# hamzalsheikh/multi-cluster-simulator

Measured on AMD Instinct MI355X. Metric: job placements/sec (whole node) at 4096 clusters x 256 nodes, higher is better.
Workload: dtype u32; 1 GPU; C4: 4096 clusters total x 256 nodes, split 4096 per GPU over 1 GPU(s) (strong sharding, clusters keyed by global index), FIFO, no trading, 16384 jobs/cluster, scaled per-second Poisson arrivals at 90% memory load (lambda=1.5386/s); clusters_total=4096, clusters_per_gpu=4096, nodes=256, jobs_per_cluster=16384, gen=stream, max_dur=600, parallelism=dp1: one system's clusters split over the GPUs, no collective on the data path

## Files before the change

### multi-cluster-simulator_amd/csrc/mcs_fa_macros.h

```cpp
#pragma once


#define MCS_FA_PRIO(P)                                                                            \
    "s_sub_u32 s76, s42, s57\n\t"                                                                 \
    "s_cselect_b32 s76, 0, s76\n\t"                                                               \
    "s_lshl_b32 s76, s76, 1\n\t"                                                                  \
    "s_cmp_gt_u32 s76, s42\n\t"                                                                   \
    "s_cbranch_scc0 " P "p2_%=\n\t"                                                              \
    "s_setprio 3\n\t"                                                                            \
    "s_branch " P "pe_%=\n"                                                                       \
    P "p2_%=:\n\t"                                                                               \
    "s_lshl_b32 s76, s76, 1\n\t"                                                                  \
    "s_cmp_gt_u32 s76, s42\n\t"                                                                   \
    "s_cbranch_scc0 " P "p1_%=\n\t"                                                              \
    "s_setprio 2\n\t"                                                                            \
    "s_branch " P "pe_%=\n"                                                                       \
    P "p1_%=:\n\t"                                                                               \
    "s_lshl_b32 s76, s76, 1\n\t"                                                                  \
    "s_cmp_gt_u32 s76, s42\n\t"                                                                   \
    "s_cbranch_scc0 " P "p0_%=\n\t"                                                              \
    "s_setprio 1\n\t"                                                                            \
    "s_branch " P "pe_%=\n"                                                                       \
    P "p0_%=:\n\t"                                                                               \
    "s_setprio 0\n"                                                                               \
// ... 297 lines not shown
#define MCS_FA_ANYFIT "v_cmp_ne_u32_e32 vcc, 0, v86\n\t"
#define MCS_FA_ANYFIT32 MCS_FA_ANYFIT
#define MCS_FA_ANYFIT16 MCS_FA_ANYFIT
#define MCS_FA_ANYFIT16R MCS_FA_ANYFIT
#define MCS_FA_PICK1 "v_readlane_b32 s51, v86, s50\n\t"
#define MCS_FA_PICK2 "s_ff1_i32_b32 s52, s51\n\t"
#define MCS_FA_PICK132 MCS_FA_PICK1
#define MCS_FA_PICK116 MCS_FA_PICK1
#define MCS_FA_PICK116R MCS_FA_PICK1
#define MCS_FA_PICK232 MCS_FA_PICK2
#define MCS_FA_PICK216 MCS_FA_PICK2
#define MCS_FA_PICK216R MCS_FA_PICK2
#define MCS_FA_ZEROKX                                                                             \
    "v_readlane_b32 s51, v86, s50\n\t"                                                           \
    "s_mov_b32 m0, s47\n\t"                                                                      \
    "s_ff1_i32_b32 s52, s51\n\t"                                                                 \
    "s_lshl3_add_u32 s54, s52, s50\n\t"
#define MCS_FA_ZEROKX32 MCS_FA_ZEROKX
#define MCS_FA_ZEROKX16 MCS_FA_ZEROKX
#define MCS_FA_ZEROKX16R MCS_FA_ZEROKX
#define MCS_FA_GUARD0_                                                                            \
    "s_mov_b32 s78, 0\n\t"                                                                        \
    "s_lshl2_add_u32 s79, s42, 0x100\n\t"
#define MCS_FA_GUARD032 MCS_FA_GUARD0_
#define MCS_FA_GUARD016 MCS_FA_GUARD0_
#define MCS_FA_GUARD016S MCS_FA_GUARD0_
#define MCS_FA_HEAD32 ""
#define MCS_FA_HEAD16 ""
#define MCS_FA_HEAD16S ""
#define MCS_FA_XWAITED_ "s_mov_b32 %[waited], s82\n\t"
#define MCS_FA_XWAITED32 MCS_FA_XWAITED_
#define MCS_FA_XWAITED16 MCS_FA_XWAITED_
#define MCS_FA_XWAITED16S MCS_FA_XWAITED_
#define MCS_FA_POOLMAX32 "64*8"
#define MCS_FA_POOLMAX16 "64*8"
#define MCS_FA_POOLMAX16R "64*8"
#define MCS_FA_NODEIDX                                                                            \
    "v_and_b32 v126, 63, v91\n\t"                                                                \
    "v_lshrrev_b32 v127, 6, v91\n\t"                                                             \
    "v_lshl_add_u32 v126, v126, 2, v127\n\t"
#define MCS_FA_NODEIDX32 MCS_FA_NODEIDX
#define MCS_FA_NODEIDX16 MCS_FA_NODEIDX
#define MCS_FA_NODEIDX16R MCS_FA_NODEIDX

#define MCS_FA_FIT16C                                                                             \
    "v_pk_sub_u16 v72, v64, s48\n\t"                                                              \
    "v_pk_sub_u16 v73, v65, s48\n\t"                                                              \
    "v_pk_sub_u16 v74, v66, s48\n\t"                                                              \
    "v_pk_sub_u16 v75, v67, s48\n\t"                                                              \
    "v_and_b32_sdwa v80, v72, v72 dst_sel:WORD_0 dst_unused:UNUSED_PAD src0_sel:WORD_1 src1_sel:WORD_0\n\t" \
    "v_and_b32_sdwa v81, v74, v74 dst_sel:WORD_0 dst_unused:UNUSED_PAD src0_sel:WORD_1 src1_sel:WORD_0\n\t" \
    "v_and_b32_sdwa v80, v73, v73 dst_sel:WORD_1 dst_unused:UNUSED_PRESERVE src0_sel:WORD_1 src1_sel:WORD_0\n\t" \
    "v_and_b32_sdwa v81, v75, v75 dst_sel:WORD_1 dst_unused:UNUSED_PRESERVE src0_sel:WORD_1 src1_sel:WORD_0\n\t" \
    "s_add_u32 s55, s40, s46\n\t"     \
    "v_perm_b32 v86, v81, v80, s72\n\t"
#define MCS_FA_REC16C MCS_FA_REC16
#define MCS_FA_ZMASK16C(SRC)                                                                      \
    "v_mov_b32 v87, " SRC "\n\t"                                                                  \
    "v_cmp_eq_u32_e32 vcc, 0, v95\n\t"                                                            \
    "v_cndmask_b32_e32 v94, " SRC ", v111, vcc\n\t"
#define MCS_FA_TAKE16C                                                                            \
    "v_mov_b32 v95, v99\n\t"                                                                      \
    "v_min_u32 v96, 0x7fff, v100\n\t"                                                             \
    "v_min_u32 v97, 0x7fff, v101\n\t"                                                             \
    "v_lshl_or_b32 v96, v97, 16, v96\n\t" MCS_FA_ZMASK16C("v98")
#define MCS_FC_SHIFT                                                                              \
    "v_cmp_le_u32_e32 vcc, s41, v110\n\t"                                                         \
    "v_cndmask_b32_e32 v94, v94, v111, vcc\n\t"                                  \
    "v_mov_b32 v89, -1\n\t"                                                                       \
    "v_mov_b32 v90, 0\n\t"                                                                        \
    "v_mov_b32 v107, 0\n\t"                                                                       \
    "s_nop 1\n\t"                                                                                 \
    "v_mov_b32_dpp v89, v94 wave_shl:1 row_mask:0xf bank_mask:0xf\n\t"                            \
    "v_mov_b32_dpp v90, v95 wave_shl:1 row_mask:0xf bank_mask:0xf\n\t"                            \
    "v_mov_b32_dpp v107, v96 wave_shl:1 row_mask:0xf bank_mask:0xf\n\t"
#define MCS_FC_RECNEXT                                                                            \
    "v_readlane_b32 s45, v89, m0\n\t"                                                             \
    "v_readlane_b32 s46, v90, m0\n\t"                                                             \
    "v_readlane_b32 s48, v107, m0\n\t"
#define MCS_FA_RELOAD16C "ds_read_b128 v[64:67], v108\n\t"
#define MCS_FA_ZEROKX16C                                                                          \
    "v_readlane_b32 s51, v86, s50\n\t"                                                           \
    "s_mov_b32 m0, s47\n\t"                                                                      \
    "s_ff1_i32_b32 s52, s51\n\t"                                                                 \
    "s_lshr_b32 s53, s52, 3\n\t"                                                                 \
    "s_lshl2_add_u32 s54, s50, s53\n\t"
#define MCS_FA_POOLMAX16C "64*8"
#define MCS_FA_NODEIDX16C "v_mov_b32 v126, v91\n\t"
#define MCS_FA_XWAITED16C                                                                         \
    "s_cmp_lg_u32 s43, 0\n\t"                                                                     \
    "s_addc_u32 %[waited], s82, 0\n\t"
#define MCS_FA_GUARD016C "s_lshl2_add_u32 s78, s42, 0x100\n\t"
#define MCS_FA_HEAD16C ""
#define MCS_FA_INIT16C MCS_FA_ZMASK16C("v94")                                      \
    "s_min_u32 s41, s42, 64\n\t" MCS_FC_SHIFT                                                     \
    "s_mov_b64 s[86:87], -1\n\t"                                                                 \
    "s_mov_b64 s[88:89], -1\n\t"                                                                 \
    "s_mov_b64 s[90:91], -1\n\t"                                                                 \
    "s_mov_b64 s[92:93], -1\n\t"                                                                 \
    "s_mov_b64 s[94:95], -1\n\t"                                                                 \
    "s_mov_b64 s[96:97], -1\n\t"                                                                 \
    "s_mov_b64 s[98:99], -1\n\t"                                                                 \
    "s_mov_b64 s[100:101], -1\n\t"                                                               \
    "s_getpc_b64 s[58:59]\n"                                                                      \
    "mcsfa_pc_%=:\n\t"                                                                            \
    "s_add_u32 s74, s58, mcsfa_tbl_%=-mcsfa_pc_%=\n\t"                                           \
    "s_addc_u32 s59, s59, 0\n\t"                                                                      \
    "v_mov_b32 v32, -1\n\t"                                                                      \
    "v_mov_b32 v33, -1\n\t"                                                                      \
    "v_mov_b32 v34, -1\n\t"                                                                      \
    "v_mov_b32 v35, -1\n\t"                                                                      \
    "v_mov_b32 v36, -1\n\t"                                                                      \
    "v_mov_b32 v37, -1\n\t"                                                                      \
    "v_mov_b32 v38, -1\n\t"                                                                      \
    "v_mov_b32 v39, -1\n\t"                                                                      \
    "v_mov_b32 v106, -1\n\t"
#define MCS_FA_DECIDE16C                                                                          \
    "v_readlane_b32 s51, v86, s50\n\t"                                                            \
    "s_lshl_b64 exec, 1, s50\n\t"                                                                 \
    "s_ff1_i32_b32 s52, s51\n\t"                                                                  \
    "s_lshr_b32 s53, s52, 3\n\t"                                                                  \
    "s_lshl2_add_u32 s54, s50, s53\n\t"              \
    "s_set_gpr_idx_on s53, gpr_idx(SRC0,DST)\n\t"                                                 \
    "v_mov_b32 v64, v72\n\t"                                 \
    "s_set_gpr_idx_off\n\t"
#define MCS_FC_BREL(P, k, F, PAY, A, FREE, TAIL)                                                  \
    "mcsfa_" P #k "_%=:\n\t"                                                                      \
    "ds_write_b128 v108, v[64:67]\n\t"                                                           \
    "s_mov_b64 exec, vcc\n\t"                                                                     \
    "s_bcnt1_i32_b64 s76, vcc\n\t"                                                               \
    "v_lshl_add_u32 v121, v91, 2, v109\n\t"                                                      \
    "ds_add_u32 v121, v96\n\t"                                                                    \
    "v_mov_b32 v106, -1\n\t"                                                                      \
    "s_mov_b64 exec, -1\n\t"                                                                      \
    "v_cmp_ge_u32_e32 vcc, s40, " F "\n\t"                                                       \
    "s_cbranch_vccz mcsfa_" TAIL #k "_%=\n\t"                                                     \
    "s_mov_b64 exec, vcc\n\t"                                                                     \
    "s_bcnt1_i32_b64 s49, vcc\n\t"                                                               \
    "ds_add_u32 " A ", " PAY "\n\t"                                                             \
    "v_mov_b32 " F ", -1\n\t"                                                                    \
    "s_or_b64 " FREE ", " FREE ", vcc\n\t"                                                       \
    "s_add_u32 s76, s76, s49\n\t"                                                                 \
    "s_branch mcsfa_" TAIL #k "_%=\n"
#define MCS_FC_BMA(r, OP, ON, FREE)                                                               \
    "v_cmp_eq_u32_e64 s[60:61], " #r ", v122\n\t"                                                 \
    "s_bcnt1_i32_b64 s76, s[60:61]\n\t"                                                           \
    "v_mbcnt_lo_u32_b32 v120, s60, v121\n\t"                                                      \
    "s_bcnt1_i32_b64 s75, " FREE "\n\t"                                                           \
    "v_mbcnt_hi_u32_b32 v120, s61, v120\n\t"                                                      \
    "s_add_u32 " ON ", " OP ", s76\n\t"                                                           \
    "v_cndmask_b32_e64 v123, v123, v120, s[60:61]\n\t"                                            \
    "s_cmp_gt_u32 s76, s75\n\t"                                                                   \
    "s_cbranch_scc1 mcsfa_bmo" #r "_%=\n"                                                         \
    "mcsfa_bmr" #r "_%=:\n\t"                                                                     \
    "v_mov_b32 v121, " ON "\n\t"
#define MCS_FC_BMO(r, OP)                                                                         \
    "mcsfa_bmo" #r "_%=:\n\t"                                                                     \
    "s_add_u32 s75, s75, " OP "\n\t"                                                              \
    "v_cmp_le_u32_e32 vcc, s75, v120\n\t"                                                         \
    "s_and_b64 vcc, vcc, s[60:61]\n\t"                                                            \
    "s_or_b64 s[46:47], s[46:47], vcc\n\t"                                                        \
    "s_branch mcsfa_bmr" #r "_%=\n"
#define MCS_FC_BMB(OP, ON, FREELO, FREEHI, FREE, Q)                                               \
    "v_mov_b32 v121, " OP "\n\t"                                                                  \
    "v_mbcnt_lo_u32_b32 v120, " FREELO ", v121\n\t"                                               \
    "v_mbcnt_hi_u32_b32 v120, " FREEHI ", v120\n\t"                                               \
    "v_cmp_gt_u32_e64 s[60:61], " ON ", v120\n\t"                                                 \
    "v_lshl_add_u32 v120, v120, 4, v109\n\t"                                                      \
    "s_and_b64 exec, s[60:61], " FREE "\n\t"                                                      \
    "ds_read_b128 " Q ", v120 offset:1024\n\t"                                                    \
    "s_andn2_b64 " FREE ", " FREE ", exec\n\t"                                                    \
    "s_mov_b64 exec, -1\n\t"
#define MCS_FC_BMC(Q0, Q1, Q2, F, P, A)                                                           \
    "v_cmp_ne_u32_e32 vcc, -1, " Q0 "\n\t"                                                        \
    "v_cndmask_b32_e32 " F ", " F ", " Q0 ", vcc\n\t"                                             \
    "v_cndmask_b32_e32 " P ", " P ", " Q1 ", vcc\n\t"                                             \
    "v_cndmask_b32_e32 " A ", " A ", " Q2 ", vcc\n\t"
#define MCS_FC_BMOVE                                                                              \
    "v_cmp_ne_u32_e32 vcc, -1, v106\n\t"                                                          \
    "s_cbranch_vccz mcsfa_bmx_%=\n\t"                                                             \
    "v_and_b32 v122, 7, v106\n\t"                                                                 \
    "s_mov_b64 s[48:49], vcc\n\t"                                            \
    "v_cndmask_b32_e32 v122, 8, v122, vcc\n\t"                      \
    "s_mov_b64 s[46:47], 0\n\t"                                                                   \
    "v_mov_b32 v112, v106\n\t"                                                                    \
    "v_mov_b32 v113, v96\n\t"                                                                     \
    "v_lshl_add_u32 v114, v91, 2, v109\n\t"                                                       \
    "v_mov_b32 v121, 0\n\t"                                                                       \
    MCS_FC_BMA(0, "0", "s50", "s[86:87]") MCS_FC_BMA(1, "s50", "s51", "s[88:89]")                 \
    MCS_FC_BMA(2, "s51", "s52", "s[90:91]") MCS_FC_BMA(3, "s52", "s53", "s[92:93]")               \
    MCS_FC_BMA(4, "s53", "s54", "s[94:95]") MCS_FC_BMA(5, "s54", "s55", "s[96:97]")               \
    MCS_FC_BMA(6, "s55", "s62", "s[98:99]") MCS_FC_BMA(7, "s62", "s63", "s[100:101]")             \
    "s_mov_b64 exec, s[48:49]\n\t"                                                                \
    "v_lshl_add_u32 v123, v123, 4, v109\n\t"                                                      \
    "ds_write_b128 v123, v[112:115] offset:1024\n\t"                                              \
    "s_mov_b64 exec, -1\n\t"                                                                      \
    "v_mov_b32 v56, -1\n\t"                                                                       \
    "v_mov_b32 v60, -1\n\t"                                                                       \
    "v_mov_b32 v68, -1\n\t"                                                                       \
    "v_mov_b32 v72, -1\n\t"                                                                       \
    "v_mov_b32 v76, -1\n\t"                                                                       \
    "v_mov_b32 v82, -1\n\t"                                                                       \
    "v_mov_b32 v102, -1\n\t"                                                                      \
    "v_mov_b32 v124, -1\n\t"                                                                      \
    MCS_FC_BMB("0", "s50", "s86", "s87", "s[86:87]", "v[56:59]")                                  \
    MCS_FC_BMB("s50", "s51", "s88", "s89", "s[88:89]", "v[60:63]")                                \
    MCS_FC_BMB("s51", "s52", "s90", "s91", "s[90:91]", "v[68:71]")                                \
    MCS_FC_BMB("s52", "s53", "s92", "s93", "s[92:93]", "v[72:75]")                                \
    MCS_FC_BMB("s53", "s54", "s94", "s95", "s[94:95]", "v[76:79]")                                \
    MCS_FC_BMB("s54", "s55", "s96", "s97", "s[96:97]", "v[82:85]")                                \
    MCS_FC_BMB("s55", "s62", "s98", "s99", "s[98:99]", "v[102:105]")                              \
    MCS_FC_BMB("s62", "s63", "s100", "s101", "s[100:101]", "v[124:127]")                          \
    "s_waitcnt lgkmcnt(0)\n\t"                                                                    \
    MCS_FC_BMC("v56", "v57", "v58", "v32", "v40", "v48")                                          \
    MCS_FC_BMC("v60", "v61", "v62", "v33", "v41", "v49")                                          \
    MCS_FC_BMC("v68", "v69", "v70", "v34", "v42", "v50")                                          \
    MCS_FC_BMC("v72", "v73", "v74", "v35", "v43", "v51")                                          \
    MCS_FC_BMC("v76", "v77", "v78", "v36", "v44", "v52")                                          \
    MCS_FC_BMC("v82", "v83", "v84", "v37", "v45", "v53")                                          \
    MCS_FC_BMC("v102", "v103", "v104", "v38", "v46", "v54")                                       \
    MCS_FC_BMC("v124", "v125", "v126", "v39", "v47", "v55")                                       \
    "s_cmp_lg_u64 s[46:47], 0\n\t"                                                                \
    "s_cbranch_scc1 mcsfa_bml_%=\n"                                                               \
    "mcsfa_bmd_%=:\n\t"                                                                           \
    "v_mov_b32 v106, -1\n"                                                                        \
    "mcsfa_bmx_%=:\n\t"
#define MCS_FC_BMOVE_OOL                                                                          \
    MCS_FC_BMO(0, "0") MCS_FC_BMO(1, "s50") MCS_FC_BMO(2, "s51") MCS_FC_BMO(3, "s52")             \
    MCS_FC_BMO(4, "s53") MCS_FC_BMO(5, "s54") MCS_FC_BMO(6, "s55") MCS_FC_BMO(7, "s62")           \
    "mcsfa_bml_%=:\n\t"                                                                           \
    "s_ff1_i32_b64 s52, s[46:47]\n\t"                                                             \
    "s_lshl_b64 s[60:61], 1, s52\n\t"                                                             \
    "v_readlane_b32 s55, v106, s52\n\t"                                              \
    "v_readlane_b32 s48, v96, s52\n\t"                                              \
    "v_readlane_b32 s54, v91, s52\n\t"                                                 \
    "s_andn2_b64 s[46:47], s[46:47], s[60:61]\n\t"                                                \
    "s_and_b32 s76, s55, 7\n\t"                                                                   \
    "s_mov_b32 s49, s76\n"                                                                        \
    "mcsfa_bms_%=:\n\t"                                                                           \
    "s_add_u32 s49, s49, 1\n\t"                                                                   \
    "s_and_b32 s49, s49, 7\n\t"                                                                   \
    "s_cmp_eq_u32 s49, s76\n\t"                                                                   \
    "s_cbranch_scc1 mcsfa_poolovf_%=\n\t"                                                         \
    "s_lshl_b32 m0, s49, 1\n\t"                                                                   \
    "s_nop 0\n\t"                                                                                 \
    "s_movrels_b64 s[60:61], s[86:87]\n\t"                                                        \
    "s_cmp_lg_u64 s[60:61], 0\n\t"                                                                \
    "s_cbranch_scc0 mcsfa_bms_%=\n\t"                                                             \
    "s_ff1_i32_b64 s85, s[60:61]\n\t"                                                             \
    "s_lshl_b64 s[62:63], 1, s85\n\t"                                                             \
    "s_andn2_b64 s[50:51], s[60:61], s[62:63]\n\t"                                                \
    "s_movreld_b64 s[86:87], s[50:51]\n\t"                                                        \
    "s_min_u32 s77, s77, s55\n\t"                                                                 \
    "s_lshl2_add_u32 s79, s54, s73\n\t"                                                           \
    "s_mov_b64 exec, s[62:63]\n\t"                                                                \
    "s_set_gpr_idx_on s49, gpr_idx(DST)\n\t"                                                      \
    "v_mov_b32 v32, s55\n\t"                                                                      \
    "v_mov_b32 v40, s48\n\t"                                                                      \
    "v_mov_b32 v48, s79\n\t"                                                                      \
    "s_set_gpr_idx_off\n\t"                                                                       \
    "s_mov_b64 exec, -1\n\t"                                                                      \
    "s_cmp_lg_u64 s[46:47], 0\n\t"                                                                \
    "s_cbranch_scc1 mcsfa_bml_%=\n\t"                                                             \
    "s_branch mcsfa_bmd_%=\n"
#define MCS_FC_WMIN(DST)                                                                          \
    "s_nop 1\n\t"                                                                                 \
    "v_min_u32_dpp v120, v120, v120 row_shr:1 row_mask:0xf bank_mask:0xf\n\t"                     \
    "s_nop 1\n\t"                                                                                 \
    "v_min_u32_dpp v120, v120, v120 row_shr:2 row_mask:0xf bank_mask:0xf\n\t"                     \
    "s_nop 1\n\t"                                                                                 \
    "v_min_u32_dpp v120, v120, v120 row_shr:4 row_mask:0xf bank_mask:0xf\n\t"                     \
    "s_nop 1\n\t"                                                                                 \
    "v_min_u32_dpp v120, v120, v120 row_shr:8 row_mask:0xf bank_mask:0xf\n\t"                     \
    "s_nop 1\n\t"                                                                                 \
    "v_min_u32_dpp v120, v120, v120 row_bcast:15 row_mask:0xa bank_mask:0xf\n\t"                  \
    "s_nop 1\n\t"                                                                                 \
    "v_min_u32_dpp v120, v120, v120 row_bcast:31 row_mask:0xc bank_mask:0xf\n\t"                  \
    "s_nop 1\n\t"                                                                                 \
    "v_readlane_b32 " DST ", v120, 63\n\t"
#define MCS_FC_FROW(p, F, P, A, FREE)                                                             \
    "v_cmp_ge_u32_e32 vcc, s40, " F "\n\t"                           \
    "s_cbranch_vccz mcsfa_fr" #p "_%=\n\t"                                                       \
    "s_mov_b64 exec, vcc\n\t"                                                                     \
    "s_bcnt1_i32_b64 s76, vcc\n\t"                                                               \
    "ds_add_u32 " A ", " P "\n\t"                                                               \
    "v_mov_b32 " F ", -1\n\t"                                                                    \
    "s_add_u32 s49, s49, s76\n\t"                                                                \
    "s_or_b64 " FREE ", " FREE ", vcc\n\t"                                                       \
    "s_mov_b64 exec, -1\n"                                                    \
    "mcsfa_fr" #p "_%=:\n\t"
#define MCS_FC_XROW(p, F)                                                                         \
    "v_and_b32 v121, 7, " F "\n\t"                                                               \
    "v_cmp_ne_u32_e32 vcc, " #p ", v121\n\t"                                                     \
    "v_cndmask_b32_e32 v121, v111, " F ", vcc\n\t"                                               \
    "v_min_u32 v120, v120, v121\n\t"
#define MCS_FC_FULL                                                                               \
    "mcsfa_full_%=:\n\t"                                                                          \
    "ds_write_b128 v108, v[64:67]\n\t"                                                           \
    "s_mov_b32 s49, 0\n\t"                                                                        \
    MCS_FC_FROW(0, "v32", "v40", "v48", "s[86:87]") MCS_FC_FROW(1, "v33", "v41", "v49", "s[88:89]") \
    MCS_FC_FROW(2, "v34", "v42", "v50", "s[90:91]") MCS_FC_FROW(3, "v35", "v43", "v51", "s[92:93]") \
    MCS_FC_FROW(4, "v36", "v44", "v52", "s[94:95]") MCS_FC_FROW(5, "v37", "v45", "v53", "s[96:97]") \
    MCS_FC_FROW(6, "v38", "v46", "v54", "s[98:99]") MCS_FC_FROW(7, "v39", "v47", "v55", "s[100:101]") \
      \
    "v_cmp_ge_u32_e32 vcc, s40, v106\n\t"                                                        \
    "s_cbranch_vccz mcsfa_fr8_%=\n\t"                                                            \
    "s_mov_b64 exec, vcc\n\t"                                                                    \
    "s_bcnt1_i32_b64 s76, vcc\n\t"                                                              \
    "v_lshl_add_u32 v121, v91, 2, v109\n\t"                                                     \
    "ds_add_u32 v121, v96\n\t"                                                                   \
    "v_mov_b32 v106, -1\n\t"                                                                     \
    "s_add_u32 s49, s49, s76\n\t"                                                                \
    "s_mov_b64 exec, -1\n"                                                                       \
    "mcsfa_fr8_%=:\n\t"                                                                          \
    "s_cmp_lt_u32 s40, s77\n\t"                     \
    "s_cbranch_scc1 mcsfa_fx_%=\n\t"                                                              \
    "v_mov_b32 v120, -1\n\t"                                                                      \
    MCS_FC_XROW(0, "v32") MCS_FC_XROW(1, "v33") MCS_FC_XROW(2, "v34") MCS_FC_XROW(3, "v35")      \
    MCS_FC_XROW(4, "v36") MCS_FC_XROW(5, "v37") MCS_FC_XROW(6, "v38") MCS_FC_XROW(7, "v39")      \
    MCS_FC_WMIN("s77") "\n"                                                                      \
    "mcsfa_fx_%=:\n\t"                                                                            \
    "s_mov_b32 s76, s49\n\t"                                                                      \
    "s_cmp_eq_u32 s49, 0\n\t"                                                                     \
    "s_cbranch_scc1 mcsfa_norel_%=\n\t"                                                           \
    "s_branch mcsfa_reltail_%=\n"
#define MCS_FC_EXACTMIN                                                                           \
    "v_min3_u32 v121, v32, v33, v34\n\t"                                                         \
    "v_min3_u32 v121, v121, v35, v36\n\t"                                                        \
    "v_min3_u32 v121, v121, v37, v38\n\t"                                                        \
    "v_min3_u32 v120, v121, v39, v106\n\t" MCS_FC_WMIN("s76")
#define MCS_FC_ZROUTE(D)                                                                          \
    "mcsfa_zarr_%=:\n\t"                                                                          \
    "s_cmp_eq_u32 s47, 64\n\t"   \
    "s_cbranch_scc1 mcsfa_bend_%=\n\t"                                                            \
    "s_add_u32 s76, s57, s47\n\t"                                                                 \
    "s_cmp_ge_u32 s76, s42\n\t"                                                                   \
    "s_cbranch_scc1 mcsfa_bend_%=\n\t"                                                            \
    "v_readlane_b32 s76, v87, s47\n\t"                                     \
    "s_cmp_lg_u32 s46, 0\n\t"                                                                     \
    "s_cselect_b32 s76, s45, s76\n\t"              \
    "s_cmp_gt_u32 s76, s40\n\t"                                                                   \
    "s_cbranch_scc0 mcsfa_zfit_%=\n\t"                                                            \
    "s_sub_u32 s49, s76, s40\n\t"                                                                 \
    "s_mov_b32 s40, s76\n\t"                                       \
    MCS_FA_CNTS_##D                                                                               \
    "s_cmp_lg_u32 s49, 1\n\t"                                                                     \
    "s_cbranch_scc1 mcsfa_full_%=\n\t"                                                            \
    "s_branch mcsfa_adv1_%=\n"                                                                    \
    "mcsfa_zfit_%=:\n\t" MCS_FA_FIT16C MCS_FA_ANYFIT                                             \
    "s_cbranch_vccz mcsfa_znofit_%=\n\t"                                                          \
    "s_ff1_i32_b64 s50, vcc\n\t"                                                                  \
    "s_branch mcsfa_zero_%=\n"                                                                    \
    "mcsfa_znofit_%=:\n\t"                                                                        \
    "s_mov_b32 s43, 2\n\t"                                                                        \
    MCS_FA_CNTS_##D                                                                               \
    "s_sub_u32 s78, s78, 1\n\t"                                           \
    "s_cbranch_scc1 mcsfa_poolovf_%=\n\t"                                                         \
    "s_cmp_eq_u32 s80, 0\n\t"                                               \
    "s_cbranch_scc1 mcsfa_deadlock_%=\n\t" MCS_FC_EXACTMIN                                        \
    "s_cmp_eq_u32 s76, -1\n\t"             \
    "s_cbranch_scc1 mcsfa_poolovf_%=\n\t"                                                         \
    "s_max_u32 s40, s40, s76\n\t"                                                                 \
    "s_branch mcsfa_full_%=\n"                                                                    \
// ... 67 lines not shown
    "s_mov_b64 exec, -1\n\t"                                                                      \
    "s_sub_u32 s80, s80, s76\n\t" MCS_FA_RELOAD16C                                               \
    "s_add_u32 s55, s40, s46\n\t"                                                    \
    "s_waitcnt lgkmcnt(0)\n\t"                                                                    \
    "v_pk_sub_u16 v72, v64, s48\n\t"                                                              \
    "v_pk_sub_u16 v73, v65, s48\n\t"                                                              \
    "v_pk_sub_u16 v74, v66, s48\n\t"                                                              \
    "v_pk_sub_u16 v75, v67, s48\n\t"                                                              \
    "v_and_b32_sdwa v80, v72, v72 dst_sel:WORD_0 dst_unused:UNUSED_PAD src0_sel:WORD_1 src1_sel:WORD_0\n\t" \
    "v_and_b32_sdwa v81, v74, v74 dst_sel:WORD_0 dst_unused:UNUSED_PAD src0_sel:WORD_1 src1_sel:WORD_0\n\t" \
    "v_and_b32_sdwa v80, v73, v73 dst_sel:WORD_1 dst_unused:UNUSED_PRESERVE src0_sel:WORD_1 src1_sel:WORD_0\n\t" \
    "v_and_b32_sdwa v81, v75, v75 dst_sel:WORD_1 dst_unused:UNUSED_PRESERVE src0_sel:WORD_1 src1_sel:WORD_0\n\t" \
    "s_cmp_le_u32 s45, s40\n\t"             \
    "v_perm_b32 v86, v81, v80, s72\n\t" MCS_FA_ANYFIT                                            \
    "s_cbranch_scc1 mcsfa_fitted" #k "_%=\n\t"                                                    \
    "s_branch mcsfa_arrive" #k "_%=\n"                                                            \
    ".p2align 6\n\t"                                                                              \
    "s_nop 0\n\t"                             \
    "s_nop 0\n"                                                                                   \
                      \
    "mcsfa_norel" #k "_%=:\n"                                                                     \
    "mcsfa_inner" #k "_%=:\n\t"                                                                   \
    "s_cmp_gt_u32 s45, s40\n\t"                          \
    "s_cbranch_scc1 mcsfa_arrive" #k "_%=\n"                                                      \
    "mcsfa_fit" #k "_%=:\n\t" MCS_FA_FIT16C MCS_FA_ANYFIT "\n"                                   \
    "mcsfa_fitted" #k "_%=:\n\t"     \
    "s_cbranch_vccz mcsfa_nofit" #k "_%=\n\t"                                                     \
    "s_ff1_i32_b64 s50, vcc\n\t"                                      \
    MCS_FA_DECIDE16C                                                                              \
    "s_mov_b64 exec, -1\n\t"                                                                      \
    "s_mov_b32 m0, s47\n\t"                                                                       \
    "s_add_u32 s80, s80, 1\n\t"                                                                   \
    "v_writelane_b32 v91, s54, m0\n\t"                                                            \
    "v_writelane_b32 v92, s40, m0\n\t"                                                            \
    "v_writelane_b32 v106, s55, m0\n"                                                               \
                                                                              \
     \
                                       \
    "mcsfa_placed" #k "_%=:\n\t" MCS_FC_RECNEXT                                                  \
    "s_add_u32 s47, s47, 1\n\t"                                                                   \
    "s_cmp_le_u32 s45, s40\n\t"                                                                   \
    "s_cbranch_scc1 mcsfa_fit" #k "_%=\n\t"                                                       \
    "s_cmp_eq_u32 s45, -1\n\t"                                                                    \
    "s_cbranch_scc1 mcsfa_zarr_%=\n"                                                              \
                  \
    "mcsfa_arr2" #k "_%=:\n\t"                                                                    \
    "s_sub_u32 s76, s45, s40\n\t"                                                                 \
    "s_mov_b32 s40, s45\n\t"                                                          \
    MCS_FA_CNTS_##D                                                                               \
    "s_cmp_lg_u32 s76, 1\n\t"                                                                     \
    "s_cbranch_scc1 mcsfa_full_%=\n\t" MCS_FC_ADV(n)                                              \
                                                \
    "mcsfa_arrive" #k "_%=:\n\t"                                                                  \
    "s_cmp_eq_u32 s45, -1\n\t"       \
    "s_cbranch_scc1 mcsfa_zarr_%=\n\t"                                                            \
    "s_branch mcsfa_arr2" #k "_%=\n"                                                              \
     \
    MCS_FC_BREL("brel", k, F, P, A, FREE, "reltail") MCS_FC_BREL("wbrel", k, F, P, A, FREE, "wreltail") \
     \
     \
       \
    "mcsfa_nofit" #k "_%=:\n\t"                                                                   \
    "s_mov_b32 s43, 1\n\t"                                                                        \
    MCS_FA_CNTS_##D                                                                               \
    "s_sub_u32 s78, s78, 1\n\t"           \
    "s_cbranch_scc1 mcsfa_poolovf_%=\n\t"                                                         \
    "s_add_u32 s79, s40, 9\n\t"                                                                   \
    "s_min_u32 s79, s79, s77\n\t"                                                                 \
    "s_cmp_eq_u32 s80, 0\n\t"                                               \
    "s_cbranch_scc0 mcsfa_wsl" #n "_%=\n\t"                                                       \
    "s_branch mcsfa_deadlock_%=\n"                                                                \
          \
    "mcsfa_wnorel" #k "_%=:\n\t"                                                                  \
    "s_add_u32 s79, s40, 9\n\t"                                                                   \
    "s_min_u32 s79, s79, s77\n\t"                                                                 \
    "s_branch mcsfa_wsl" #n "_%=\n"                                                               \
      \
      \
    "mcsfa_wrel" #k "_%=:\n\t"                                                                    \
    "ds_write_b128 v108, v[64:67]\n\t"                                                           \
    "s_mov_b64 exec, vcc\n\t"                                                                     \
    "s_bcnt1_i32_b64 s76, vcc\n\t"                                                               \
    "ds_add_u32 " A ", " P "\n\t"                                                               \
    "v_mov_b32 " F ", -1\n\t"                                                                    \
    "s_or_b64 " FREE ", " FREE ", vcc\n"                                                         \
    "mcsfa_wreltail" #k "_%=:\n\t" MCS_FA_CNTR_##D                                               \
    "s_max_u32 s81, s81, s80\n\t"                                                                 \
    "s_mov_b64 exec, -1\n\t"                                                                      \
    "s_sub_u32 s80, s80, s76\n\t" MCS_FA_RELOAD16C                                               \
    "s_waitcnt lgkmcnt(0)\n\t" MCS_FA_FIT16C MCS_FA_ANYFIT                                       \
    "s_cbranch_vccz mcsfa_nofit" #k "_%=\n\t"      \
         \
        \
                                      \
    "s_ff1_i32_b64 s50, vcc\n\t"                                                                  \
    MCS_FA_DECIDE16C                                                                              \
    "s_mov_b64 exec, -1\n\t"                                                                      \
    "s_mov_b32 m0, s47\n\t"                                                                       \
    "s_add_u32 s80, s80, 1\n\t"                                                                   \
    "v_writelane_b32 v91, s54, m0\n\t"                                                            \
    "v_writelane_b32 v92, s40, m0\n\t"                                                            \
    "v_writelane_b32 v106, s55, m0\n\t"                                                            \
    "s_add_u32 s82, s82, 1\n\t"                                                                   \
    "s_mov_b32 s43, 0\n\t" MCS_FC_RECNEXT                                                        \
    "s_add_u32 s47, s47, 1\n\t"                                                                   \
    "s_add_u32 s40, s40, 1\n\t"                                                                   \
    "s_cmp_ge_u32 s40, s77\n\t"                                                                   \
    "s_cbranch_scc1 mcsfa_full_%=\n" TAIL
#define MCS_FC_WSL(k, F)                                                                          \
    "mcsfa_wsl" #k "_%=:\n\t"                                                                     \
    "s_add_u32 s40, s40, 1\n\t"                                                                   \
    "s_cmp_ge_u32 s40, s79\n\t"                                                                   \
    "s_cbranch_scc1 mcsfa_wslow_%=\n"                                                             \
    "mcsfa_wblk" #k "_%=:\n\t"                                                                    \
    "v_cmp_ge_u32_e32 vcc, s40, v106\n\t"                                                        \
    "s_cbranch_vccnz mcsfa_wbrel" #k "_%=\n\t"                                                    \
    "v_cmp_ge_u32_e32 vcc, s40, " F "\n\t"                                                       \
    "s_cbranch_vccnz mcsfa_wrel" #k "_%=\n"
#define MCS_FC_PASS(D)                                                                            \
    "s_branch mcsfa_inner_%=\n"                                                                   \
    ".p2align 6\n"                                                                                \
    MCS_FC_COPY(D, 0, 1, "v32", "v40", "v48", "s[86:87]", "")                                     \
    MCS_FC_COPY(D, 1, 2, "v33", "v41", "v49", "s[88:89]", "")                                     \
    MCS_FC_COPY(D, 2, 3, "v34", "v42", "v50", "s[90:91]", "")                                     \
    MCS_FC_COPY(D, 3, 4, "v35", "v43", "v51", "s[92:93]", "")                                     \
    MCS_FC_COPY(D, 4, 5, "v36", "v44", "v52", "s[94:95]", "")                                     \
    MCS_FC_COPY(D, 5, 6, "v37", "v45", "v53", "s[96:97]", "")                                     \
    MCS_FC_COPY(D, 6, 7, "v38", "v46", "v54", "s[98:99]", "")                                     \
    MCS_FC_COPY(D, 7, 0, "v39", "v47", "v55", "s[100:101]", "\ts_branch mcsfa_blk0_%=\n")         \
                                     \
    MCS_FC_WSL(0, "v32") MCS_FC_WSL(1, "v33") MCS_FC_WSL(2, "v34") MCS_FC_WSL(3, "v35")           \
    MCS_FC_WSL(4, "v36") MCS_FC_WSL(5, "v37") MCS_FC_WSL(6, "v38") MCS_FC_WSL(7, "v39")           \
    "\ts_branch mcsfa_wsl0_%=\n"                                                                  \
                                                                  \
     \
            \
    "mcsfa_wslow_%=:\n\t"                                                                         \
    "s_cmp_ge_u32 s40, s77\n\t"                                                                   \
    "s_cbranch_scc1 mcsfa_full_%=\n"                                                              \
    "mcsfa_exact_%=:\n\t" MCS_FC_EXACTMIN                                                         \
    "s_cmp_eq_u32 s76, -1\n\t"             \
    "s_cbranch_scc1 mcsfa_poolovf_%=\n\t"                                                         \
    "s_max_u32 s40, s40, s76\n\t"                                                                 \
    "s_add_u32 s79, s40, 9\n\t"                                                                   \
    "s_min_u32 s79, s79, s77\n\t"                                                                 \
    "s_cmp_ge_u32 s40, s77\n\t"                                                                   \
    "s_cbranch_scc1 mcsfa_full_%=\n\t" MCS_FC_RET("s49", 7)                                      \
     \
                                          \
    "mcsfa_zero_%=:\n\t" MCS_FA_ZEROKX16C                                                        \
    "v_writelane_b32 v91, s54, m0\n\t"                                                            \
    "v_writelane_b32 v92, s40, m0\n\t"                                                            \
    "s_cmp_lg_u32 s43, 0\n\t"                                                                     \
    "s_cbranch_scc1 mcsfa_zhead_%=\n\t" MCS_FC_RET("s49", 9)                                    \
     \
                                                            \
    "mcsfa_adv1_%=:\n\t"                                                                          \
    "s_cmp_ge_u32 s40, s77\n\t"                                                                   \
    "s_cbranch_scc1 mcsfa_full_%=\n\t" MCS_FC_RET("s49", 0)                                      \
    "mcsfa_norel_%=:\n\t" MCS_FC_RETW("s49", 1)                                                  \
    "mcsfa_reltail_%=:\n\t" MCS_FC_RETW("s49", 4)                                                \
    "mcsfa_inner_%=:\n\t" MCS_FC_RET("s49", 8)                                                  \
    MCS_FC_FULL MCS_FC_ZROUTE(D)                                                     \
    ".p2align 9\n"                                                                                \
    "mcsfa_tbl_%=:\n\t" MCS_FC_TBL("blk") MCS_FC_TBL("norel") MCS_FC_TBL("wnorel")               \
// ... 81 lines not shown
```

### multi-cluster-simulator_amd/csrc/mcs_fifo_asm.hip

```cpp
#include "mcs_gen_dev.h"
#include "mcs_internal.h"
#include "mcs_lds.h"
#include "mcs_wave.h"

namespace mcs {

namespace {

#ifdef MCS_STAMPS
__device__ unsigned long long g_fa_stamps[4];
#endif

#include "mcs_fa_macros.h"

#define MCS_FA_ENTRY_S(W)                                                                         \
                                            \
    "s_mov_b32 s40, %[t]\n\t"                                                                     \
    "s_mov_b32 s42, %[J]\n\t"                                                                     \
    "s_mov_b32 s43, 0\n\t"                                                                        \
    "s_mov_b32 s44, 0\n\t"                                                                        \
    "s_mov_b32 s47, 0\n\t"                                                                        \
    "s_mov_b32 s57, 0\n\t" MCS_FA_GUARD0##W                                                      \
    "s_mov_b32 s80, 0\n\t"                                                                        \
    "s_mov_b32 s81, 0\n\t"                                                                        \
// ... 100 lines not shown
                            \
    MCS_FA_CNTR_##D MCS_FA_T0                                                                     \
    "s_max_u32 s81, s81, s80\n\t"                    \
    "s_add_u32 s74, s40, 1\n\t"                           \
    MCS_FA_SCAN##W MCS_FA_SCANEND MCS_FA_T1("s94")                                               \
                            \
    "s_cmp_lt_u32 s47, s41\n\t"                                                                   \
    "s_cbranch_scc1 mcsfa_inner_%=\n\t"                                                           \
    "s_branch mcsfa_loopend_%=\n" MCS_FA_RBODY##W

#define MCS_FA_ENDS(W, F)                                                                         \
    "mcsfa_deadlock_%=:\n\t"                                                                      \
    "s_or_b32 s44, s44, %[fdl]\n\t"                                                               \
    "s_branch mcsfa_exit_%=\n"                                                                    \
    "mcsfa_clkovf_%=:\n\t"                                                                        \
    "s_mov_b32 s40, -1\n\t"                    \
    "s_or_b32 s44, s44, %[fck]\n\t"                                                               \
    "s_branch mcsfa_exit_%=\n"                                                                    \
    "mcsfa_poolovf_%=:\n\t"                                                                       \
    "s_or_b32 s44, s44, %[fov]\n\t"                                                               \
    "s_branch mcsfa_exit_%=\n"                                                                    \
                                                                                                  \
     \
    "mcsfa_bend_%=:\n\t" MCS_FA_T0                                                               \
    "s_max_u32 s81, s81, s80\n\t"                                                                 \
    "s_cmp_gt_u32 s81, " MCS_FA_POOLMAX##W "\n\t"                                                 \
    "s_cbranch_scc1 mcsfa_poolovf_%=\n\t"                                                         \
    "s_add_u32 s76, s57, s47\n\t"                                                                 \
    "s_cmp_ge_u32 s76, s42\n\t"                                                                   \
    "s_cbranch_scc1 mcsfa_exit_%=\n\t"                                                            \
    "s_waitcnt vmcnt(0)\n\t"                                                                      \
    "v_add_u32 v125, s57, v110\n\t"                                                               \
    "v_lshlrev_b32 v125, 2, v125\n\t"                                                             \
    MCS_FA_NODEIDX##W                                                                             \
    "global_store_dword v125, v126, s[66:67] nt\n\t"                                              \
    "global_store_dword v125, v92, s[68:69] nt\n\t"                                               \
    "v_add_u32 v93, v92, v95\n\t"             \
    "global_store_dword v125, v93, s[70:71] nt\n\t"                                               \
    "s_add_u32 s57, s57, 64\n\t" MCS_FA_PRIO("mcsfa_") MCS_FA_BENDTAIL_##F(W)

#define MCS_FA_BODY(W, D, F) MCS_FA_PASS(W, D) MCS_FA_ENDS(W, F)

#define MCS_FA_BENDTAIL_S(W)                                                                      \
    MCS_FA_TAKE##W                                                                                \
    "v_add_u32 v121, s57, v110\n\t"                                                               \
    "v_lshlrev_b32 v121, 4, v121\n\t"                                                             \
    "v_add_u32 v121, 0x400, v121\n\t"                                                             \
    "global_load_dwordx4 v[98:101], v121, s[64:65]\n\t"                                           \
    "s_sub_u32 s41, s42, s57\n\t"                                                                 \
    "s_min_u32 s41, s41, 64\n\t"                                                                  \
    "s_mov_b32 s47, 0\n\t" MCS_FA_REC##W MCS_FA_T1("s96")                                         \
    "s_branch mcsfa_inner_%=\n"
#define MCS_FA_BENDTAIL_C(W)                                                                      \
    MCS_FC_BMOVE                                                                                  \
    "s_sub_u32 s41, s42, s57\n\t"                                                                 \
    "s_min_u32 s41, s41, 64\n\t" MCS_FA_TAKE##W                                                   \
    "v_add_u32 v121, s57, v110\n\t"                                                               \
    "v_lshlrev_b32 v121, 4, v121\n\t"                                                             \
    "v_add_u32 v121, 0x400, v121\n\t"                                                             \
    "global_load_dwordx4 v[98:101], v121, s[64:65]\n\t" MCS_FC_SHIFT                              \
    "s_mov_b32 s47, 0\n\t" MCS_FA_REC##W                                                          \
    "s_branch mcsfa_inner_%=\n" MCS_FC_BMOVE_OOL
#define MCS_FA_BENDTAIL_F(W)                                                                      \
    "s_mov_b32 s47, 0\n\t"                                                                        \
    "s_mov_b32 s59, 1\n\t" MCS_FA_T1("s96")                                                      \
    "s_branch mcsfa_exit_%=\n"

#define MCS_FA_EXIT_S(W)                                                                          \
                                     \
    "mcsfa_exit_%=:\n\t"                                                                          \
    "s_waitcnt vmcnt(0) lgkmcnt(0)\n\t" MCS_FA_TEND                                               \
    "s_mov_b32 %[t], s40\n\t"                                                                     \
    "s_add_u32 %[r], s57, s47\n\t"                                                                \
    "s_mov_b32 %[flags], s44\n\t"                                                                 \
    "s_mov_b32 %[hw], s43\n\t"                                                                    \
    "s_mov_b32 %[used], s80\n\t"                                                                  \
    "s_max_u32 %[peak], s81, s80\n\t"                                                             \
    MCS_FA_XWAITED##W                                                                             \
    "s_mov_b32 %[nslow], s83\n\t"                                                                 \
    "s_mov_b32 %[nrel], s84\n\t"                                                                  \
    "v_mov_b32 %[on], v91\n\t"                                                                    \
    "v_mov_b32 %[os], v92\n\t"                                                                    \
     \
      \
               \
    "s_cmp_eq_u32 s47, 0\n\t"                                                                     \
    "s_cbranch_scc1 mcsfa_xf_%=\n\t"                                                              \
    "v_add_u32 v93, v92, v95\n"                                                                   \
    "mcsfa_xf_%=:\n\t"                                                                            \
    "v_mov_b32 %[of], v93\n\t"                                                                    \
    "v_mov_b32 %[frm], v89\n\t"                                                                   \
    "v_mov_b32 %[lmin], v90\n\t"                                                                  \
    "s_nop 1"

#define MCS_FA_LOOP(W, D) MCS_FA_ENTRY_S(W) MCS_FA_BODY(W, D, S) MCS_FA_EXIT_S(W)
#define MCS_FC_LOOP(D) MCS_FA_ENTRY_S(16C) MCS_FC_PASS(D) MCS_FA_ENDS(16C, C) MCS_FA_EXIT_S(16C)
#define MCS_FC_CLOBBERS                                                                                      \
    MCS_FA_CLOBBERS, "s92", "s93", "s94", "s95", "s96", "s97", "s98", "s99", "s100", "s101", "v56", "v57", "v58", \
        "v59", "v60", "v61", "v62", "v63", "v102", "v103", "v104", "v105", "v106"

#define MCS_FA_ENTRY_F(W)                                                                         \
    "s_mov_b32 s42, %[J]\n\t"                                                                     \
    "s_lshl2_add_u32 s79, s42, 0x100\n\t"                                                         \
    "s_mov_b64 s[66:67], %[onp]\n\t"                                                              \
    "s_mov_b64 s[68:69], %[osp]\n\t"                                                              \
    "s_mov_b64 s[70:71], %[ofp]\n\t"                                                              \
    "s_mov_b32 s72, %[sel0]\n\t"                                                                  \
    "s_mov_b32 s73, %[sel1]\n\t"                                                                  \
    "s_mov_b32 s49, 0x100\n\t"                                                                    \
    "v_mov_b32 v107, %[pay]\n\t"                                                                  \
    "v_mov_b32 v108, %[nb]\n\t"                                                                   \
    "v_mov_b32 v109, %[nbase]\n\t"                                                                \
    "v_mov_b32 v110, %[lane]\n\t"                                                                 \
    "v_mov_b32 v111, -1\n\t"                                                                      \
    "s_cmp_eq_u32 s59, 0\n\t"                                                                     \
    "s_mov_b32 s59, 0\n\t"                                                   \
    "s_cbranch_scc0 mcsfa_resume_%=\n\t" MCS_FA_INIT##W MCS_FA_RELOAD##W                         \
    "v_mov_b32 v94, %[c0]\n\t"                                                                    \
    "v_mov_b32 v95, %[c1]\n\t"                                                                    \
    "v_mov_b32 v96, %[c2]\n\t"                                                                    \
    "v_mov_b32 v97, %[c3]\n\t"                                                                    \
    "s_waitcnt lgkmcnt(0)\n\t"                                                                    \
    "s_min_u32 s41, s42, 64\n\t"                                                                  \
    "s_branch mcsfa_start_%=\n"                                                                   \
    "mcsfa_resume_%=:\n\t" MCS_FA_TAKE##W                                                        \
    "s_sub_u32 s41, s42, s57\n\t"                                                                 \
    "s_min_u32 s41, s41, 64\n\t"                                                                  \
    "s_mov_b32 s47, 0\n"                                                                          \
    "mcsfa_start_%=:\n\t" MCS_FA_REC##W                                                          \
    "s_cmp_lt_u32 s47, s41\n\t"                                                                   \
    "s_cbranch_scc0 mcsfa_bend_%=\n"
#define MCS_FA_EXIT_F                                                                             \
// ... 326 lines not shown
```

Measured before the change: 15.62 billion placements/s.

## Interleave per-slot heap triples in VGPRs and derive start time lazily

Each slot's three-field record (finish, payload, address) now lives in one contiguous 4-register group (v32..v35, v36..v39, ...) instead of three separate 8-register arrays. The batch-move path can then ds_read_b128 straight into the final registers, dropping the scratch registers and the per-slot conditional-select merge sequence, and indirect writes use one scaled index. Per-placement writelanes of the start time into v92 are removed; start is recomputed as finish minus duration at release/store time through a new STARTS hook. This cuts instructions in the hot loop and frees VGPRs (v102-v105) from the clobber list. The risk is subtle correctness in the recomputed start and in the register remapping.

Measured after the change: 16.09 billion placements/s, median of 6. +3.0%, better.

```diff
diff --git a/multi-cluster-simulator_amd/csrc/mcs_fa_macros.h b/multi-cluster-simulator_amd/csrc/mcs_fa_macros.h
--- a/multi-cluster-simulator_amd/csrc/mcs_fa_macros.h
+++ b/multi-cluster-simulator_amd/csrc/mcs_fa_macros.h
@@ -353,6 +353,10 @@
 #define MCS_FA_XWAITED32 MCS_FA_XWAITED_
 #define MCS_FA_XWAITED16 MCS_FA_XWAITED_
 #define MCS_FA_XWAITED16S MCS_FA_XWAITED_
+#define MCS_FA_STARTS32 ""
+#define MCS_FA_STARTS16 ""
+#define MCS_FA_STARTS16S ""
+#define MCS_FA_STARTS16R ""
 #define MCS_FA_POOLMAX32 "64*8"
 #define MCS_FA_POOLMAX16 "64*8"
 #define MCS_FA_POOLMAX16R "64*8"
@@ -408,6 +412,10 @@
     "s_lshl2_add_u32 s54, s50, s53\n\t"
 #define MCS_FA_POOLMAX16C "64*8"
 #define MCS_FA_NODEIDX16C "v_mov_b32 v126, v91\n\t"
+#define MCS_FA_STARTS16C                                                                          \
+    "v_cmp_ne_u32_e32 vcc, -1, v106\n\t"                                                          \
+    "v_sub_u32 v120, v106, v95\n\t"                                                               \
+    "v_cndmask_b32_e32 v92, v92, v120, vcc\n\t"
 #define MCS_FA_XWAITED16C                                                                         \
     "s_cmp_lg_u32 s43, 0\n\t"                                                                     \
     "s_addc_u32 %[waited], s82, 0\n\t"
@@ -428,13 +436,13 @@
     "s_add_u32 s74, s58, mcsfa_tbl_%=-mcsfa_pc_%=\n\t"                                           \
     "s_addc_u32 s59, s59, 0\n\t"                                                                      \
     "v_mov_b32 v32, -1\n\t"                                                                      \
-    "v_mov_b32 v33, -1\n\t"                                                                      \
-    "v_mov_b32 v34, -1\n\t"                                                                      \
-    "v_mov_b32 v35, -1\n\t"                                                                      \
     "v_mov_b32 v36, -1\n\t"                                                                      \
-    "v_mov_b32 v37, -1\n\t"                                                                      \
-    "v_mov_b32 v38, -1\n\t"                                                                      \
-    "v_mov_b32 v39, -1\n\t"                                                                      \
+    "v_mov_b32 v40, -1\n\t"                                                                      \
+    "v_mov_b32 v44, -1\n\t"                                                                      \
+    "v_mov_b32 v48, -1\n\t"                                                                      \
+    "v_mov_b32 v52, -1\n\t"                                                                      \
+    "v_mov_b32 v56, -1\n\t"                                                                      \
+    "v_mov_b32 v60, -1\n\t"                                                                      \
     "v_mov_b32 v106, -1\n\t"
 #define MCS_FA_DECIDE16C                                                                          \
     "v_readlane_b32 s51, v86, s50\n\t"                                                            \
@@ -452,6 +460,7 @@
     "s_bcnt1_i32_b64 s76, vcc\n\t"                                                               \
     "v_lshl_add_u32 v121, v91, 2, v109\n\t"                                                      \
     "ds_add_u32 v121, v96\n\t"                                                                    \
+    "v_sub_u32 v92, v106, v95\n\t"                  \
     "v_mov_b32 v106, -1\n\t"                                                                      \
     "s_mov_b64 exec, -1\n\t"                                                                      \
     "v_cmp_ge_u32_e32 vcc, s40, " F "\n\t"                                                       \
@@ -492,11 +501,6 @@
     "ds_read_b128 " Q ", v120 offset:1024\n\t"                                                    \
     "s_andn2_b64 " FREE ", " FREE ", exec\n\t"                                                    \
     "s_mov_b64 exec, -1\n\t"
-#define MCS_FC_BMC(Q0, Q1, Q2, F, P, A)                                                           \
-    "v_cmp_ne_u32_e32 vcc, -1, " Q0 "\n\t"                                                        \
-    "v_cndmask_b32_e32 " F ", " F ", " Q0 ", vcc\n\t"                                             \
-    "v_cndmask_b32_e32 " P ", " P ", " Q1 ", vcc\n\t"                                             \
-    "v_cndmask_b32_e32 " A ", " A ", " Q2 ", vcc\n\t"
 #define MCS_FC_BMOVE                                                                              \
     "v_cmp_ne_u32_e32 vcc, -1, v106\n\t"                                                          \
     "s_cbranch_vccz mcsfa_bmx_%=\n\t"                                                             \
@@ -516,31 +520,15 @@
     "v_lshl_add_u32 v123, v123, 4, v109\n\t"                                                      \
     "ds_write_b128 v123, v[112:115] offset:1024\n\t"                                              \
     "s_mov_b64 exec, -1\n\t"                                                                      \
-    "v_mov_b32 v56, -1\n\t"                                                                       \
-    "v_mov_b32 v60, -1\n\t"                                                                       \
-    "v_mov_b32 v68, -1\n\t"                                                                       \
-    "v_mov_b32 v72, -1\n\t"                                                                       \
-    "v_mov_b32 v76, -1\n\t"                                                                       \
-    "v_mov_b32 v82, -1\n\t"                                                                       \
-    "v_mov_b32 v102, -1\n\t"                                                                      \
-    "v_mov_b32 v124, -1\n\t"                                                                      \
-    MCS_FC_BMB("0", "s50", "s86", "s87", "s[86:87]", "v[56:59]")                                  \
-    MCS_FC_BMB("s50", "s51", "s88", "s89", "s[88:89]", "v[60:63]")                                \
-    MCS_FC_BMB("s51", "s52", "s90", "s91", "s[90:91]", "v[68:71]")                                \
-    MCS_FC_BMB("s52", "s53", "s92", "s93", "s[92:93]", "v[72:75]")                                \
-    MCS_FC_BMB("s53", "s54", "s94", "s95", "s[94:95]", "v[76:79]")                                \
-    MCS_FC_BMB("s54", "s55", "s96", "s97", "s[96:97]", "v[82:85]")                                \
-    MCS_FC_BMB("s55", "s62", "s98", "s99", "s[98:99]", "v[102:105]")                              \
-    MCS_FC_BMB("s62", "s63", "s100", "s101", "s[100:101]", "v[124:127]")                          \
+    MCS_FC_BMB("0", "s50", "s86", "s87", "s[86:87]", "v[32:35]")                                  \
+    MCS_FC_BMB("s50", "s51", "s88", "s89", "s[88:89]", "v[36:39]")                                \
+    MCS_FC_BMB("s51", "s52", "s90", "s91", "s[90:91]", "v[40:43]")                                \
+    MCS_FC_BMB("s52", "s53", "s92", "s93", "s[92:93]", "v[44:47]")                                \
+    MCS_FC_BMB("s53", "s54", "s94", "s95", "s[94:95]", "v[48:51]")                                \
+    MCS_FC_BMB("s54", "s55", "s96", "s97", "s[96:97]", "v[52:55]")                                \
+    MCS_FC_BMB("s55", "s62", "s98", "s99", "s[98:99]", "v[56:59]")                                \
+    MCS_FC_BMB("s62", "s63", "s100", "s101", "s[100:101]", "v[60:63]")                            \
     "s_waitcnt lgkmcnt(0)\n\t"                                                                    \
-    MCS_FC_BMC("v56", "v57", "v58", "v32", "v40", "v48")                                          \
-    MCS_FC_BMC("v60", "v61", "v62", "v33", "v41", "v49")                                          \
-    MCS_FC_BMC("v68", "v69", "v70", "v34", "v42", "v50")                                          \
-    MCS_FC_BMC("v72", "v73", "v74", "v35", "v43", "v51")                                          \
-    MCS_FC_BMC("v76", "v77", "v78", "v36", "v44", "v52")                                          \
-    MCS_FC_BMC("v82", "v83", "v84", "v37", "v45", "v53")                                          \
-    MCS_FC_BMC("v102", "v103", "v104", "v38", "v46", "v54")                                       \
-    MCS_FC_BMC("v124", "v125", "v126", "v39", "v47", "v55")                                       \
     "s_cmp_lg_u64 s[46:47], 0\n\t"                                                                \
     "s_cbranch_scc1 mcsfa_bml_%=\n"                                                               \
     "mcsfa_bmd_%=:\n\t"                                                                           \
@@ -574,11 +562,12 @@
     "s_movreld_b64 s[86:87], s[50:51]\n\t"                                                        \
     "s_min_u32 s77, s77, s55\n\t"                                                                 \
     "s_lshl2_add_u32 s79, s54, s73\n\t"                                                           \
+    "s_lshl_b32 s75, s49, 2\n\t"                                 \
     "s_mov_b64 exec, s[62:63]\n\t"                                                                \
-    "s_set_gpr_idx_on s49, gpr_idx(DST)\n\t"                                                      \
+    "s_set_gpr_idx_on s75, gpr_idx(DST)\n\t"                                                      \
     "v_mov_b32 v32, s55\n\t"                                                                      \
-    "v_mov_b32 v40, s48\n\t"                                                                      \
-    "v_mov_b32 v48, s79\n\t"                                                                      \
+    "v_mov_b32 v33, s48\n\t"                                                                      \
+    "v_mov_b32 v34, s79\n\t"                                                                      \
     "s_set_gpr_idx_off\n\t"                                                                       \
     "s_mov_b64 exec, -1\n\t"                                                                      \
     "s_cmp_lg_u64 s[46:47], 0\n\t"                                                                \
@@ -619,10 +608,10 @@
     "mcsfa_full_%=:\n\t"                                                                          \
     "ds_write_b128 v108, v[64:67]\n\t"                                                           \
     "s_mov_b32 s49, 0\n\t"                                                                        \
-    MCS_FC_FROW(0, "v32", "v40", "v48", "s[86:87]") MCS_FC_FROW(1, "v33", "v41", "v49", "s[88:89]") \
-    MCS_FC_FROW(2, "v34", "v42", "v50", "s[90:91]") MCS_FC_FROW(3, "v35", "v43", "v51", "s[92:93]") \
-    MCS_FC_FROW(4, "v36", "v44", "v52", "s[94:95]") MCS_FC_FROW(5, "v37", "v45", "v53", "s[96:97]") \
-    MCS_FC_FROW(6, "v38", "v46", "v54", "s[98:99]") MCS_FC_FROW(7, "v39", "v47", "v55", "s[100:101]") \
+    MCS_FC_FROW(0, "v32", "v33", "v34", "s[86:87]") MCS_FC_FROW(1, "v36", "v37", "v38", "s[88:89]") \
+    MCS_FC_FROW(2, "v40", "v41", "v42", "s[90:91]") MCS_FC_FROW(3, "v44", "v45", "v46", "s[92:93]") \
+    MCS_FC_FROW(4, "v48", "v49", "v50", "s[94:95]") MCS_FC_FROW(5, "v52", "v53", "v54", "s[96:97]") \
+    MCS_FC_FROW(6, "v56", "v57", "v58", "s[98:99]") MCS_FC_FROW(7, "v60", "v61", "v62", "s[100:101]") \
       \
     "v_cmp_ge_u32_e32 vcc, s40, v106\n\t"                                                        \
     "s_cbranch_vccz mcsfa_fr8_%=\n\t"                                                            \
@@ -630,6 +619,7 @@
     "s_bcnt1_i32_b64 s76, vcc\n\t"                                                              \
     "v_lshl_add_u32 v121, v91, 2, v109\n\t"                                                     \
     "ds_add_u32 v121, v96\n\t"                                                                   \
+    "v_sub_u32 v92, v106, v95\n\t"                                                \
     "v_mov_b32 v106, -1\n\t"                                                                     \
     "s_add_u32 s49, s49, s76\n\t"                                                                \
     "s_mov_b64 exec, -1\n"                                                                       \
@@ -637,8 +627,8 @@
     "s_cmp_lt_u32 s40, s77\n\t"                     \
     "s_cbranch_scc1 mcsfa_fx_%=\n\t"                                                              \
     "v_mov_b32 v120, -1\n\t"                                                                      \
-    MCS_FC_XROW(0, "v32") MCS_FC_XROW(1, "v33") MCS_FC_XROW(2, "v34") MCS_FC_XROW(3, "v35")      \
-    MCS_FC_XROW(4, "v36") MCS_FC_XROW(5, "v37") MCS_FC_XROW(6, "v38") MCS_FC_XROW(7, "v39")      \
+    MCS_FC_XROW(0, "v32") MCS_FC_XROW(1, "v36") MCS_FC_XROW(2, "v40") MCS_FC_XROW(3, "v44")      \
+    MCS_FC_XROW(4, "v48") MCS_FC_XROW(5, "v52") MCS_FC_XROW(6, "v56") MCS_FC_XROW(7, "v60")      \
     MCS_FC_WMIN("s77") "\n"                                                                      \
     "mcsfa_fx_%=:\n\t"                                                                            \
     "s_mov_b32 s76, s49\n\t"                                                                      \
@@ -646,10 +636,10 @@
     "s_cbranch_scc1 mcsfa_norel_%=\n\t"                                                           \
     "s_branch mcsfa_reltail_%=\n"
 #define MCS_FC_EXACTMIN                                                                           \
-    "v_min3_u32 v121, v32, v33, v34\n\t"                                                         \
-    "v_min3_u32 v121, v121, v35, v36\n\t"                                                        \
-    "v_min3_u32 v121, v121, v37, v38\n\t"                                                        \
-    "v_min3_u32 v120, v121, v39, v106\n\t" MCS_FC_WMIN("s76")
+    "v_min3_u32 v121, v32, v36, v40\n\t"                                                         \
+    "v_min3_u32 v121, v121, v44, v48\n\t"                                                        \
+    "v_min3_u32 v121, v121, v52, v56\n\t"                                                        \
+    "v_min3_u32 v120, v121, v60, v106\n\t" MCS_FC_WMIN("s76")
 #define MCS_FC_ZROUTE(D)                                                                          \
     "mcsfa_zarr_%=:\n\t"                                                                          \
     "s_cmp_eq_u32 s47, 64\n\t"   \
@@ -783,7 +773,6 @@
     "s_mov_b32 m0, s47\n\t"                                                                       \
     "s_add_u32 s80, s80, 1\n\t"                                                                   \
     "v_writelane_b32 v91, s54, m0\n\t"                                                            \
-    "v_writelane_b32 v92, s40, m0\n\t"                                                            \
     "v_writelane_b32 v106, s55, m0\n"                                                               \
                                                                               \
      \
@@ -850,7 +839,6 @@
     "s_mov_b32 m0, s47\n\t"                                                                       \
     "s_add_u32 s80, s80, 1\n\t"                                                                   \
     "v_writelane_b32 v91, s54, m0\n\t"                                                            \
-    "v_writelane_b32 v92, s40, m0\n\t"                                                            \
     "v_writelane_b32 v106, s55, m0\n\t"                                                            \
     "s_add_u32 s82, s82, 1\n\t"                                                                   \
     "s_mov_b32 s43, 0\n\t" MCS_FC_RECNEXT                                                        \
@@ -871,17 +859,17 @@
 #define MCS_FC_PASS(D)                                                                            \
     "s_branch mcsfa_inner_%=\n"                                                                   \
     ".p2align 6\n"                                                                                \
-    MCS_FC_COPY(D, 0, 1, "v32", "v40", "v48", "s[86:87]", "")                                     \
-    MCS_FC_COPY(D, 1, 2, "v33", "v41", "v49", "s[88:89]", "")                                     \
-    MCS_FC_COPY(D, 2, 3, "v34", "v42", "v50", "s[90:91]", "")                                     \
-    MCS_FC_COPY(D, 3, 4, "v35", "v43", "v51", "s[92:93]", "")                                     \
-    MCS_FC_COPY(D, 4, 5, "v36", "v44", "v52", "s[94:95]", "")                                     \
-    MCS_FC_COPY(D, 5, 6, "v37", "v45", "v53", "s[96:97]", "")                                     \
-    MCS_FC_COPY(D, 6, 7, "v38", "v46", "v54", "s[98:99]", "")                                     \
-    MCS_FC_COPY(D, 7, 0, "v39", "v47", "v55", "s[100:101]", "\ts_branch mcsfa_blk0_%=\n")         \
+    MCS_FC_COPY(D, 0, 1, "v32", "v33", "v34", "s[86:87]", "")                                     \
+    MCS_FC_COPY(D, 1, 2, "v36", "v37", "v38", "s[88:89]", "")                                     \
+    MCS_FC_COPY(D, 2, 3, "v40", "v41", "v42", "s[90:91]", "")                                     \
+    MCS_FC_COPY(D, 3, 4, "v44", "v45", "v46", "s[92:93]", "")                                     \
+    MCS_FC_COPY(D, 4, 5, "v48", "v49", "v50", "s[94:95]", "")                                     \
+    MCS_FC_COPY(D, 5, 6, "v52", "v53", "v54", "s[96:97]", "")                                     \
+    MCS_FC_COPY(D, 6, 7, "v56", "v57", "v58", "s[98:99]", "")                                     \
+    MCS_FC_COPY(D, 7, 0, "v60", "v61", "v62", "s[100:101]", "\ts_branch mcsfa_blk0_%=\n")         \
                                      \
-    MCS_FC_WSL(0, "v32") MCS_FC_WSL(1, "v33") MCS_FC_WSL(2, "v34") MCS_FC_WSL(3, "v35")           \
-    MCS_FC_WSL(4, "v36") MCS_FC_WSL(5, "v37") MCS_FC_WSL(6, "v38") MCS_FC_WSL(7, "v39")           \
+    MCS_FC_WSL(0, "v32") MCS_FC_WSL(1, "v36") MCS_FC_WSL(2, "v40") MCS_FC_WSL(3, "v44")           \
+    MCS_FC_WSL(4, "v48") MCS_FC_WSL(5, "v52") MCS_FC_WSL(6, "v56") MCS_FC_WSL(7, "v60")           \
     "\ts_branch mcsfa_wsl0_%=\n"                                                                  \
                                                                   \
      \
diff --git a/multi-cluster-simulator_amd/csrc/mcs_fifo_asm.hip b/multi-cluster-simulator_amd/csrc/mcs_fifo_asm.hip
--- a/multi-cluster-simulator_amd/csrc/mcs_fifo_asm.hip
+++ b/multi-cluster-simulator_amd/csrc/mcs_fifo_asm.hip
@@ -156,7 +156,7 @@
     "s_waitcnt vmcnt(0)\n\t"                                                                      \
     "v_add_u32 v125, s57, v110\n\t"                                                               \
     "v_lshlrev_b32 v125, 2, v125\n\t"                                                             \
-    MCS_FA_NODEIDX##W                                                                             \
+    MCS_FA_NODEIDX##W MCS_FA_STARTS##W                                                            \
     "global_store_dword v125, v126, s[66:67] nt\n\t"                                              \
     "global_store_dword v125, v92, s[68:69] nt\n\t"                                               \
     "v_add_u32 v93, v92, v95\n\t"             \
@@ -202,7 +202,7 @@
     "s_max_u32 %[peak], s81, s80\n\t"                                                             \
     MCS_FA_XWAITED##W                                                                             \
     "s_mov_b32 %[nslow], s83\n\t"                                                                 \
-    "s_mov_b32 %[nrel], s84\n\t"                                                                  \
+    "s_mov_b32 %[nrel], s84\n\t" MCS_FA_STARTS##W                                                 \
     "v_mov_b32 %[on], v91\n\t"                                                                    \
     "v_mov_b32 %[os], v92\n\t"                                                                    \
      \
@@ -221,7 +221,7 @@
 #define MCS_FC_LOOP(D) MCS_FA_ENTRY_S(16C) MCS_FC_PASS(D) MCS_FA_ENDS(16C, C) MCS_FA_EXIT_S(16C)
 #define MCS_FC_CLOBBERS                                                                                      \
     MCS_FA_CLOBBERS, "s92", "s93", "s94", "s95", "s96", "s97", "s98", "s99", "s100", "s101", "v56", "v57", "v58", \
-        "v59", "v60", "v61", "v62", "v63", "v102", "v103", "v104", "v105", "v106"
+        "v59", "v60", "v61", "v62", "v63", "v106"
 
 #define MCS_FA_ENTRY_F(W)                                                                         \
     "s_mov_b32 s42, %[J]\n\t"                                                                     \
```
